# autosome-ru/pasio

Hardware: NVIDIA B200
Metric: whole-contig segmentation throughput, default pasio pipeline (nt/s); DP cell updates/s in dp_cells_per_s (higher is better)
Workload: dtype f64

## Files before the change

### include/pasio_b200.h

```cpp
#ifndef PASIO_B200_H
#define PASIO_B200_H

#include <stdint.h>

#ifdef __cplusplus
extern "C" {
#endif

typedef struct pasio_ctx pasio_ctx;

typedef enum pasio_status {
    PASIO_OK = 0,
    PASIO_E_CUDA = -1,
    PASIO_E_ARG = -2,
    PASIO_E_COUNTS = -3,
    PASIO_E_CANDIDATES = -4,
    PASIO_E_TABLE_TOO_SHORT = -5,
    PASIO_E_STATE = -6,
    PASIO_E_TOO_LARGE = -7,
    PASIO_E_NOMEM = -8
} pasio_status;

enum { PASIO_TAB_LOG = 0,
       PASIO_TAB_LGAMMA = 1,
// ... 26 lines not shown

int pasio_contig_load(pasio_ctx *ctx, const int64_t *counts, int64_t n,
                      const int64_t *offsets, int64_t n_contigs);
int pasio_contig_load_rle(pasio_ctx *ctx, const int64_t *starts, const int64_t *values,
                          int64_t n_runs, const int64_t *offsets, int64_t n_contigs);
int pasio_contig_load_round(pasio_ctx *ctx, const int64_t *counts, int64_t n, int64_t window_size,
                            int64_t window_shift, int constraint, int64_t *n_in, int64_t *n_out, int64_t *cells);

int pasio_contig_load_device(pasio_ctx *ctx, const int64_t *d_counts_device, int64_t n,
                             const int64_t *offsets, int64_t n_contigs);
int pasio_contig_info(const pasio_ctx *ctx, int64_t *n, int64_t *total_count, int64_t *n_contigs);
int pasio_cumsum_at(pasio_ctx *ctx, const int64_t *positions, int64_t m, int64_t *out);

int pasio_candidates_set(pasio_ctx *ctx, const int64_t *cands, int64_t m);
int pasio_candidates_count(const pasio_ctx *ctx, int64_t *m);
int pasio_candidates_download(pasio_ctx *ctx, int64_t *out, int64_t capacity, int64_t *m);

int pasio_filter_candidates(pasio_ctx *ctx, int constraint, int64_t *n_in, int64_t *n_out);

int pasio_round(pasio_ctx *ctx, int64_t window_size, int64_t window_shift, int constraint,
                int64_t *n_in, int64_t *n_out, int64_t *cells);
int pasio_round_stats(const pasio_ctx *ctx, int64_t *cells, int64_t *cells_skipped);
int pasio_round_certify_stats(const pasio_ctx *ctx, int64_t *passed, int64_t *fell_back, int64_t *resume_rows_sum);
int pasio_exact_task_plan(int64_t n_candidates, int lag, int nblock, int32_t *triples, int64_t cap, int64_t *n_tasks);
int pasio_upload_stats(const pasio_ctx *ctx, int64_t *wire_bytes);
int pasio_set_tuning(pasio_ctx *ctx, int key, int value);
int pasio_rounds(pasio_ctx *ctx, int64_t window_size, int64_t window_shift, int constraint,
                 int64_t max_rounds, int64_t *rounds_done, int64_t *n_out, int64_t *cells,
                 int64_t *sizes, int64_t sizes_cap);
int pasio_set_penalties(pasio_ctx *ctx, const double *split_number_penalty, int64_t n_split_number_penalty,
                        double first_column_refund, const double *length_penalty, int64_t n_length_penalty);

int pasio_square_split(pasio_ctx *ctx, int64_t *out_splits, int64_t cap, int64_t *n_splits,
                       double *score, double *prefix_scores, int64_t *previous_splits);
int pasio_square_split_regularized(pasio_ctx *ctx, const double *length_penalty, int64_t n_length_penalty,
                                   const double *split_number_penalty, int64_t n_split_number_penalty,
                                   double first_column_refund, int64_t *out_splits, int64_t cap, int64_t *n_splits,
                                   double *score, double *prefix_scores, int64_t *previous_splits);
int pasio_suffix_scores(pasio_ctx *ctx, int64_t stop, double *out);

int pasio_segment_scores(pasio_ctx *ctx, double *scores, int64_t *segment_counts,
                         double *mean_counts, double *logfac_cumsum, int64_t capacity,
                         int64_t *n_segments);

int pasio_segment_scores_sum(pasio_ctx *ctx, double *total);

// ... 32 lines not shown
```

### pasio_b200/_native.py

```python
import ctypes
import os
import threading

import numpy as np

_HERE = os.path.dirname(os.path.abspath(__file__))
LIB_PATH = os.environ.get('PASIO_B200_LIB') or os.path.join(_HERE, 'libpasio_b200.so')

OK = 0
E_CUDA, E_ARG, E_COUNTS, E_CANDIDATES, E_TABLE_TOO_SHORT, E_STATE, E_TOO_LARGE, E_NOMEM = range(-1, -9, -1)
TAB_LOG, TAB_LGAMMA, TAB_LGAMMA_ALPHA = 0, 1, 2
CONSTRAINTS = {'none': 0, 'zeros': 1, 'constants': 2}
TUNE = {'window_prune': 0, 'window_phases': 1, 'exact_prune': 2, 'exact_lag': 3, 'exact_ring': 4, 'logfac_exact': 5,
        'window_speculate': 6, 'upload_narrow': 7,
        'logfac_eager': 8, 'exact_nblock': 9, 'window_certify': 10}
TIMING_FAMILIES = ['scan', 'window_dp', 'compact', 'exact_dp', 'score', 'h2d', 'd2h']

_i64 = ctypes.c_int64
_i64p = ctypes.POINTER(ctypes.c_int64)
_f64p = ctypes.POINTER(ctypes.c_double)
_vp = ctypes.c_void_p

SIGNATURES = {
    'pasio_ctx_create': (ctypes.c_int, [ctypes.c_int, ctypes.POINTER(_vp)]),
    'pasio_ctx_destroy': (ctypes.c_int, [_vp]),
    'pasio_last_error': (ctypes.c_char_p, [_vp]),
    'pasio_abi_version': (ctypes.c_int, []),
    'pasio_set_params': (ctypes.c_int, [_vp, ctypes.c_int, ctypes.c_double, ctypes.c_double, ctypes.c_double]),
    'pasio_table_upload': (ctypes.c_int, [_vp, ctypes.c_int, _f64p, _i64]),
    'pasio_table_need': (ctypes.c_int, [_vp, _i64p, _i64p, _i64p]),
    'pasio_contig_load': (ctypes.c_int, [_vp, _i64p, _i64, _i64p, _i64]),
    'pasio_contig_load_round': (ctypes.c_int, [_vp, _i64p, _i64, _i64, _i64, ctypes.c_int, _i64p, _i64p, _i64p]),
    'pasio_contig_load_rle': (ctypes.c_int, [_vp, _i64p, _i64p, _i64, _i64p, _i64]),
    'pasio_contig_load_device': (ctypes.c_int, [_vp, _vp, _i64, _i64p, _i64]),
    'pasio_contig_info': (ctypes.c_int, [_vp, _i64p, _i64p, _i64p]),
    'pasio_cumsum_at': (ctypes.c_int, [_vp, _i64p, _i64, _i64p]),
    'pasio_candidates_set': (ctypes.c_int, [_vp, _i64p, _i64]),
    'pasio_candidates_count': (ctypes.c_int, [_vp, _i64p]),
    'pasio_candidates_download': (ctypes.c_int, [_vp, _i64p, _i64, _i64p]),
    'pasio_filter_candidates': (ctypes.c_int, [_vp, ctypes.c_int, _i64p, _i64p]),
    'pasio_round': (ctypes.c_int, [_vp, _i64, _i64, ctypes.c_int, _i64p, _i64p, _i64p]),
    'pasio_round_stats': (ctypes.c_int, [_vp, _i64p, _i64p]),
    'pasio_round_certify_stats': (ctypes.c_int, [_vp, _i64p, _i64p, _i64p]),
    'pasio_exact_task_plan': (ctypes.c_int, [_i64, ctypes.c_int, ctypes.c_int, ctypes.POINTER(ctypes.c_int32), _i64, _i64p]),
    'pasio_upload_stats': (ctypes.c_int, [_vp, _i64p]),
    'pasio_set_tuning': (ctypes.c_int, [_vp, ctypes.c_int, ctypes.c_int]),
    'pasio_rounds': (ctypes.c_int, [_vp, _i64, _i64, ctypes.c_int, _i64, _i64p, _i64p, _i64p, _i64p, _i64]),
    'pasio_set_penalties': (ctypes.c_int, [_vp, _f64p, _i64, ctypes.c_double, _f64p, _i64]),
    'pasio_square_split': (ctypes.c_int, [_vp, _i64p, _i64, _i64p, _f64p, _f64p, _i64p]),
    'pasio_square_split_regularized': (ctypes.c_int, [_vp, _f64p, _i64, _f64p, _i64, ctypes.c_double, _i64p, _i64, _i64p, _f64p,
                                                     _f64p, _i64p]),
    'pasio_suffix_scores': (ctypes.c_int, [_vp, _i64, _f64p]),
    'pasio_segment_scores': (ctypes.c_int, [_vp, _f64p, _i64p, _f64p, _f64p, _i64, _i64p]),
    'pasio_segment_scores_sum': (ctypes.c_int, [_vp, _f64p]),
    'pasio_segment_lmm': (ctypes.c_int, [_vp, _f64p, _i64, _f64p]),
    'pasio_logfac_prefetch': (ctypes.c_int, [_vp]),
    'pasio_host_alloc': (ctypes.c_int, [_i64, ctypes.POINTER(_vp)]),
    'pasio_host_free': (ctypes.c_int, [_vp]),
    'pasio_bedgraph_count_lines': (_i64, [ctypes.c_void_p, _i64]),
    'pasio_bedgraph_parse': (ctypes.c_int, [ctypes.c_void_p, _i64, _i64, _i64p, _i64p, _i64p, _i64p,
                                            ctypes.POINTER(ctypes.c_int32), ctypes.POINTER(ctypes.c_uint8), _i64p, _i64p]),
    'pasio_bedgraph_runs': (_i64, [_i64p, _i64p, _i64p, ctypes.POINTER(ctypes.c_uint8), _i64, ctypes.c_int, _i64p, _i64p, _i64p,
                                   _i64p, _i64p]),
    'pasio_format_segments': (_i64, [ctypes.c_char_p, _i64, _i64p, _i64, _f64p, _f64p, ctypes.c_int,
                                     ctypes.c_char_p, _i64]),
    'pasio_format_segments_batch': (_i64, [ctypes.c_char_p, _i64p, _i64p, _i64p, _i64, _i64p, _f64p, _f64p, ctypes.c_int,
# ... 312 lines not shown
        self._sync_penalties()
        self._retry(lambda: self.lib.pasio_round(self.ctx, window_size, window_shift, CONSTRAINTS[constraint],
                                                 ctypes.byref(n_in), ctypes.byref(n_out), ctypes.byref(cells)))
        return n_in.value, n_out.value, cells.value

    def set_tuning(self, key, value):
        self._check(self.lib.pasio_set_tuning(self.ctx, TUNE[key], int(value)))

    def upload_stats(self):
        b = _i64(0)
        self._check(self.lib.pasio_upload_stats(self.ctx, ctypes.byref(b)))
        return b.value

    def round_stats(self):
        a, b = _i64(0), _i64(0)
        self._check(self.lib.pasio_round_stats(self.ctx, ctypes.byref(a), ctypes.byref(b)))
        return a.value, b.value

    def round_certify_stats(self):
        a, b, c = _i64(0), _i64(0), _i64(0)
        self._check(self.lib.pasio_round_certify_stats(self.ctx, ctypes.byref(a), ctypes.byref(b), ctypes.byref(c)))
        return a.value, b.value, c.value

    def rounds(self, window_size, window_shift, constraint, num_rounds=None, first=None):
        n, _, _ = self.info()
        limit = max(1, n if num_rounds is None else num_rounds)
        self._cands_obj = None
        sizes, cells_total = [], 0
        if first is not None:
            sizes.append(first[0])
            cells_total += first[2]
            limit -= 1
            if first[0] == first[1] or limit == 0:
                return sizes, self.candidate_count(), cells_total
        while limit > 0:
            done, n_out, cells = _i64(0), _i64(0), _i64(0)
            buf = np.zeros(64, dtype=np.int64)
            step = min(limit, 64)
            self._sync_penalties()
            rc = self.lib.pasio_rounds(self.ctx, window_size, window_shift, CONSTRAINTS[constraint], step,
                                       ctypes.byref(done), ctypes.byref(n_out), ctypes.byref(cells),
                                       _ptr(buf, ctypes.c_int64), len(buf))
            sizes.extend(buf[:done.value].tolist())
            cells_total += cells.value
            limit -= done.value
            if rc == E_TABLE_TOO_SHORT:
# ... 224 lines not shown
```

### pasio_b200/csrc/api.cu

```cuda
#include "common.cuh"

#include <algorithm>
#include <thread>
#include <atomic>
#include <chrono>
#include <memory>
#include <cstdarg>
#include <cstdlib>
#include <cstdio>
#include <cstring>

static thread_local std::string g_create_error;

int pasio_fail(pasio_ctx *ctx, int code, const char *fmt, ...)
{
    char buf[512];
    va_list ap;
    va_start(ap, fmt);
    vsnprintf(buf, sizeof buf, fmt, ap);
    va_end(ap);
    if (ctx) ctx->err = buf; else g_create_error = buf;
    return code;
}

// ... 364 lines not shown
        return pasio_fail(nullptr, PASIO_E_ARG, "device %d out of range (have %d)", device, count);
    cudaDeviceProp prop;
    e = cudaGetDeviceProperties(&prop, device);
    if (e != cudaSuccess) return pasio_fail(nullptr, PASIO_E_CUDA, "cudaGetDeviceProperties: %s", cudaGetErrorString(e));
    if (prop.major != 10)
        return pasio_fail(nullptr, PASIO_E_CUDA, "device %d is sm_%d%d; this library is built for sm_100a only",
                          device, prop.major, prop.minor);
    e = cudaSetDevice(device);
    if (e != cudaSuccess) return pasio_fail(nullptr, PASIO_E_CUDA, "cudaSetDevice: %s", cudaGetErrorString(e));
    pasio_ctx *ctx = new pasio_ctx();
    ctx->device = device;
    ctx->sm_count = prop.multiProcessorCount;
    ctx->smem_optin = (int)prop.sharedMemPerBlockOptin;
    int prio_lo = 0, prio_hi = 0;
    cudaDeviceGetStreamPriorityRange(&prio_lo, &prio_hi);
    if (cudaStreamCreateWithPriority(&ctx->stream, cudaStreamNonBlocking, prio_hi) != cudaSuccess ||
        cudaStreamCreateWithPriority(&ctx->stream2, cudaStreamNonBlocking, 0) != cudaSuccess ||
        cudaStreamCreateWithFlags(&ctx->stream_copy, cudaStreamNonBlocking) != cudaSuccess ||
        cudaStreamCreateWithPriority(&ctx->stream_lx, cudaStreamNonBlocking, 0) != cudaSuccess ||
        cudaEventCreateWithFlags(&ctx->ev_lx0, cudaEventDisableTiming) != cudaSuccess ||
        cudaEventCreateWithFlags(&ctx->ev_lx1, cudaEventDisableTiming) != cudaSuccess ||
        cudaEventCreateWithFlags(&ctx->ev_fork, cudaEventDisableTiming) != cudaSuccess ||
        cudaEventCreateWithFlags(&ctx->ev_join, cudaEventDisableTiming) != cudaSuccess ||
        cudaMallocHost((void **)&ctx->h_scalars, 20 * sizeof(i64)) != cudaSuccess ||
        pasio_reserve(ctx, ctx->scalars, 20 * sizeof(i64)) != PASIO_OK) {
        g_create_error = "context allocation failed: " + ctx->err;
        delete ctx;
        return PASIO_E_CUDA;
    }
    memset(ctx->h_scalars, 0, 20 * sizeof(i64));
    auto env_int = [](const char *name, int dflt) { const char *v = getenv(name); return v ? atoi(v) : dflt; };
    ctx->tune[PASIO_TUNE_WINDOW_PRUNE] = env_int("PASIO_WD_PRUNE", 1);
    ctx->tune[PASIO_TUNE_WINDOW_PHASES] = env_int("PASIO_WD_PHASES", 1);
    ctx->tune[PASIO_TUNE_EXACT_PRUNE] = env_int("PASIO_XD_PRUNE", 1);
    ctx->tune[PASIO_TUNE_EXACT_LAG] = env_int("PASIO_XD_LAG", 5);
    ctx->tune[PASIO_TUNE_EXACT_RING] = env_int("PASIO_XD_RING", 1);
    ctx->tune[PASIO_TUNE_LOGFAC_EXACT] = env_int("PASIO_B200_EXACT_LMM", 1);
    ctx->tune[PASIO_TUNE_WINDOW_SPECULATE] = env_int("PASIO_WD_SPECULATE", 1);
    ctx->tune[PASIO_TUNE_UPLOAD_NARROW] = env_int("PASIO_B200_UPLOAD_NARROW", 1);
    ctx->tune[PASIO_TUNE_LOGFAC_EAGER] = env_int("PASIO_B200_LOGFAC_EAGER", 0);
    ctx->tune[PASIO_TUNE_EXACT_NBLOCK] = env_int("PASIO_XD_NBLOCK", 3);
    ctx->tune[PASIO_TUNE_WINDOW_CERTIFY] = env_int("PASIO_WD_CERTIFY", 1);
    if (ctx->tune[PASIO_TUNE_EXACT_LAG] < 3 || ctx->tune[PASIO_TUNE_EXACT_LAG] > 5) ctx->tune[PASIO_TUNE_EXACT_LAG] = 5;
    *out = ctx;
    return PASIO_OK;
}

extern "C" int pasio_ctx_destroy(pasio_ctx *ctx)
{
    if (!ctx) return PASIO_OK;
    cudaSetDevice(ctx->device);
    cudaStreamSynchronize(ctx->stream);
    drop_borrowed_counts(ctx);
// ... 384 lines not shown
    if (ctx->h_scalars[1]) return pasio_fail(ctx, PASIO_E_COUNTS, "counts must be >= 0");
    ctx->total = ctx->h_scalars[0];
    ctx->max_count = ctx->h_scalars[2];
    ctx->have_contig = true;
    if (eager) {
        CUDA_TRY(ctx, cudaEventRecord(ctx->ev_lx1, ctx->stream_lx));
        ctx->logfac_ready = true;
        ctx->logfac_is_exact = true;
        ctx->logfac_pending = true;
        ctx->logfac_eager = true;
    }
    PASIO_TRY(launch_boundary_ranks(ctx));
    ctx->h_brank = ctx->h_bounds;
    if (n_in) *n_in = ctx->m;
    if (n_out) *n_out = ctx->m;
    if (cells) *cells = 0;
    if (table_rc != PASIO_OK) return table_rc;

    const int nxt = 1 - ctx->cur;
    PASIO_TRY(pasio_reserve(ctx, ctx->cand[nxt], (size_t)ctx->m * 4));
    i64 m_new = 0;
    PASIO_TRY(launch_compact_keepbits(ctx, nxt, &m_new));
    PASIO_TRY(d2h(ctx, ctx->h_scalars + 10, ctx->scalars.as<i64>() + 10, 24));
    PASIO_TRY(d2h(ctx, ctx->h_scalars + 16, ctx->scalars.as<i64>() + 16, 24));
    if (cells) *cells = ctx->h_scalars[10];
    ctx->last_cells = ctx->h_scalars[10];
    ctx->last_cells_skipped = ctx->h_scalars[12];
    for (int k = 0; k < 3; ++k) ctx->last_certify[k] = ctx->h_scalars[16 + k];
    ctx->prev_round_in = ctx->m;
    ctx->prev_round_out = m_new;
    ctx->cur = nxt;
    ctx->implicit_all = false;
    ctx->m = m_new;
    if (n_out) *n_out = m_new;
    return refresh_boundary_ranks(ctx);
}

extern "C" int pasio_contig_info(const pasio_ctx *ctx, int64_t *n, int64_t *total_count, int64_t *n_contigs)
{
    if (!ctx || !ctx->have_contig) return PASIO_E_STATE;
    if (n) *n = ctx->n;
    if (total_count) *total_count = ctx->total;
    if (n_contigs) *n_contigs = ctx->n_contigs;
    return PASIO_OK;
}

extern "C" int pasio_cumsum_at(pasio_ctx *ctx, const int64_t *positions, int64_t m, int64_t *out)
{
    NEED_CTX(ctx);
    if (!ctx->have_contig) return pasio_fail(ctx, PASIO_E_STATE, "no contig loaded");
    if (m < 0 || !out) return pasio_fail(ctx, PASIO_E_ARG, "bad arguments");
// ... 163 lines not shown
    static const bool debug = getenv("PASIO_DEBUG") != nullptr;
    if (debug)
        fprintf(stderr, "[pasio_round] n=%lld contigs=%lld m=%lld implicit=%d nwin=%lld size=%lld shift=%lld max_span=%lld max_cnt=%lld ntab=%lld,%lld,%lld\n",
                (long long)ctx->n, (long long)ctx->n_contigs, (long long)ctx->m, (int)ctx->implicit_all, (long long)nwin,
                (long long)window_size, (long long)window_shift, (long long)max_span, (long long)max_cnt,
                (long long)ctx->ntab[0], (long long)ctx->ntab[1], (long long)ctx->ntab[2]);
    if (max_cnt > ctx->total || max_span > ctx->n)
        return pasio_fail(ctx, PASIO_E_CUDA, "internal inconsistency before the window DP: window count %lld / span %lld exceed "
                          "contig total %lld / length %lld (m=%lld, implicit=%d, windows=%lld)", (long long)max_cnt,
                          (long long)max_span, (long long)ctx->total, (long long)ctx->n, (long long)ctx->m,
                          (int)ctx->implicit_all, (long long)nwin);
    PASIO_TRY(check_dp_tables(ctx, max_span, max_cnt, true));

    const size_t bit_bytes = (size_t)((ctx->n + 1 + 31) / 32 + 2) * 4;
    CUDA_TRY(ctx, cudaMemsetAsync(ctx->keepbits.p, 0, bit_bytes, ctx->stream));
    if (penalties_on(ctx)) PASIO_TRY(launch_window_dp_reg(ctx, nwin, (int)window_size, (int)window_shift, constraint));
    else PASIO_TRY(launch_window_dp(ctx, nwin, (int)window_size, (int)window_shift, constraint));

    const int nxt = 1 - ctx->cur;
    PASIO_TRY(pasio_reserve(ctx, ctx->cand[nxt], (size_t)ctx->m * 4));
    i64 m_new = 0;
    PASIO_TRY(launch_compact_keepbits(ctx, nxt, &m_new));
    PASIO_TRY(d2h(ctx, ctx->h_scalars + 10, ctx->scalars.as<i64>() + 10, 24));
    PASIO_TRY(d2h(ctx, ctx->h_scalars + 16, ctx->scalars.as<i64>() + 16, 24));
    if (cells) *cells = ctx->h_scalars[10];
    ctx->last_cells = ctx->h_scalars[10];
    ctx->last_cells_skipped = ctx->h_scalars[12];
    for (int k = 0; k < 3; ++k) ctx->last_certify[k] = ctx->h_scalars[16 + k];
    ctx->prev_round_in = ctx->m;
    ctx->prev_round_out = m_new;
    ctx->cur = nxt;
    ctx->implicit_all = false;
    ctx->m = m_new;
    if (n_out) *n_out = m_new;
    return refresh_boundary_ranks(ctx);
}

extern "C" int pasio_rounds(pasio_ctx *ctx, int64_t window_size, int64_t window_shift, int constraint,
                            int64_t max_rounds, int64_t *rounds_done, int64_t *n_out, int64_t *cells,
                            int64_t *sizes, int64_t sizes_cap)
{
    NEED_CTX(ctx);
    if (!ctx->have_contig) return pasio_fail(ctx, PASIO_E_STATE, "no contig loaded");
    i64 limit = max_rounds <= 0 ? ctx->n : max_rounds;
    if (limit < 1) limit = 1;
    i64 done = 0, total_cells = 0;
    int rc = PASIO_OK;
    while (done < limit) {
        int64_t a = 0, b = 0, c = 0;
        rc = pasio_round(ctx, window_size, window_shift, constraint, &a, &b, &c);
        if (rc != PASIO_OK) break;
// ... 9 lines not shown
}

extern "C" int pasio_upload_stats(const pasio_ctx *ctx, int64_t *wire_bytes)
{
    if (!ctx || !wire_bytes) return PASIO_E_ARG;
    *wire_bytes = ctx->last_wire_bytes;
    return PASIO_OK;
}

extern "C" int pasio_round_stats(const pasio_ctx *ctx, int64_t *cells, int64_t *cells_skipped)
{
    if (!ctx) return PASIO_E_ARG;
    if (cells) *cells = ctx->last_cells;
    if (cells_skipped) *cells_skipped = ctx->last_cells_skipped;
    return PASIO_OK;
}

extern "C" int pasio_round_certify_stats(const pasio_ctx *ctx, int64_t *passed, int64_t *fell_back, int64_t *resume_rows_sum)
{
    if (!ctx) return PASIO_E_ARG;
    if (passed) *passed = ctx->last_certify[0];
    if (fell_back) *fell_back = ctx->last_certify[1];
    if (resume_rows_sum) *resume_rows_sum = ctx->last_certify[2];
    return PASIO_OK;
}

extern "C" int pasio_set_tuning(pasio_ctx *ctx, int key, int value)
{
    if (!ctx) return PASIO_E_ARG;
    if (key < 0 || key >= PASIO_TUNE_COUNT) return pasio_fail(ctx, PASIO_E_ARG, "unknown tuning key %d", key);
    if (key == PASIO_TUNE_EXACT_LAG && (value < 3 || value > 5)) return pasio_fail(ctx, PASIO_E_ARG, "exact lag must be 3, 4 or 5");
    ctx->tune[key] = value;
    if (key == PASIO_TUNE_LOGFAC_EXACT) {
        if (ctx->logfac_pending) { cudaStreamSynchronize(ctx->stream_lx); ctx->logfac_pending = false; }
        ctx->logfac_ready = false;
        ctx->logfac_eager = false;
    }
    return PASIO_OK;
}

static int finish_square_split(pasio_ctx *ctx, i64 N, int64_t *out_splits, int64_t cap, int64_t *n_splits, double *score,
                               double *prefix_scores, int64_t *previous_splits)
{
    if (score) PASIO_TRY(d2h(ctx, score, ctx->dpP.as<double>() + (N - 1), 8));
    if (prefix_scores) PASIO_TRY(d2h(ctx, prefix_scores, ctx->dpP.p, (size_t)N * 8));
    if (previous_splits) {
// ... 335 lines not shown
```

### pasio_b200/csrc/common.cuh

```cuda
#pragma once

#include <cuda_runtime.h>
#include <stdint.h>
#include <string>
#include <vector>

#include "../../include/pasio_b200.h"

typedef long long i64;
typedef unsigned long long u64;

#define PASIO_ABI_VERSION 1

struct DevBuf {
    void *p = nullptr;
    size_t bytes = 0;
    template <typename T> T *as() const { return reinterpret_cast<T *>(p); }
};

enum TimingFamily { TF_SCAN = 0, TF_WINDOW_DP = 1, TF_COMPACT = 2, TF_EXACT_DP = 3, TF_SCORE = 4,
                    TF_H2D = 5, TF_D2H = 6, TF_COUNT = 7 };

struct TimedSpan { int family; cudaEvent_t a, b; };

// ... 54 lines not shown

    DevBuf win_st, win_en;
    DevBuf win_flags;
    DevBuf win_small, win_medium, win_large;
    i64 n_small = 0, n_medium = 0, n_large = 0;
    i64 n_large_p1 = 0;
    std::vector<int32_t> h_win_st, h_win_en, h_brank;

    DevBuf blocksum, tilestate, scalars, dpL, dpC, dpP, dpPrev, dpPart, dpPartArg, dpMark, dpJump, fscan, logfac_full;
    DevBuf xpRing, xpRec, xpTasks, regLR, regNR;

    bool pen_num = false, pen_len = false;
    DevBuf penNR, penLR;
    i64 n_pen_nr = 0, n_pen_lr = 0;
    double pen_refund = 0.0;
    DevBuf lxPos, lxSum, lxFirst, lxState;
    i64 lx_terms = 0;
    i64 scan_tiles_done = 0;

    int tune[PASIO_TUNE_COUNT];
    i64 *h_scalars = nullptr;

    i64 last_cells = 0, last_cells_skipped = 0;
    i64 last_certify[3] = {0, 0, 0};
    i64 prev_round_in = 0, prev_round_out = 0;
    std::vector<i64> pw_leaf_start;
    i64 pw_n = -1;
    std::vector<double> pw_leaf_sum;

    bool timing = false;
    std::vector<TimedSpan> spans;
    std::vector<cudaEvent_t> event_pool;
    double fam_ms[TF_COUNT] = {0};
    i64 fam_launches[TF_COUNT] = {0};
};

int pasio_fail(pasio_ctx *ctx, int code, const char *fmt, ...);
int pasio_reserve(pasio_ctx *ctx, DevBuf &b, size_t bytes);

#define CUDA_TRY(ctx, call)                                                                     \
    do {                                                                                        \
        cudaError_t e__ = (call);                                                               \
        if (e__ != cudaSuccess)                                                                 \
            return pasio_fail((ctx), PASIO_E_CUDA, "%s failed: %s (%s:%d)", #call,              \
                              cudaGetErrorString(e__), __FILE__, __LINE__);                     \
    } while (0)

// ... 92 lines not shown
```

### pasio_b200/csrc/window_dp.cu

```cuda
#include "dp_core.cuh"
#include "bound.cuh"
#include <cstdio>
#include <cstdlib>

namespace {

constexpr int WD_THREADS = 256;
constexpr int WD_WARPS = WD_THREADS / 32;
constexpr int WD_FARW = WD_WARPS - 1;
constexpr int NEAR_Q = 4;
constexpr int PR_CB = 32;
constexpr int PR_FB = 8;
constexpr int PR_MIN_N = 256;
constexpr int PR_DENSE = 28;

#ifdef PASIO_WD_PROF
__device__ unsigned long long g_wd_prof[16];
struct ProfAcc { long long t0; long long a0, a1, a2, a3, a4, a5, a6, a7; };
#define PROF_DECL ProfAcc prof = {clock64(), 0, 0, 0, 0, 0, 0, 0, 0}
__device__ __forceinline__ long long prof_clock()
{
    unsigned dummy;
    long long t;
    asm volatile("ld.volatile.shared.u32 %0, [%1];" : "=r"(dummy) : "r"(0u) : "memory");
    asm volatile("mov.u64 %0, %%clock64;" : "=l"(t) : "r"(dummy) : "memory");
    return t;
}
#define PROF_T(i) do { const long long t1__ = prof_clock(); prof.a##i += t1__ - prof.t0; prof.t0 = t1__; } while (0)
#define PROF_FLUSH do { if (threadIdx.x == 0 || threadIdx.x == 32) { unsigned long long *g__ = g_wd_prof + (threadIdx.x ? 8 : 0); \
    atomicAdd(g__ + 0, (unsigned long long)prof.a0); atomicAdd(g__ + 1, (unsigned long long)prof.a1); \
    atomicAdd(g__ + 2, (unsigned long long)prof.a2); atomicAdd(g__ + 3, (unsigned long long)prof.a3); \
    atomicAdd(g__ + 4, (unsigned long long)prof.a4); atomicAdd(g__ + 5, (unsigned long long)prof.a5); \
    atomicAdd(g__ + 6, (unsigned long long)prof.a6); atomicAdd(g__ + 7, (unsigned long long)prof.a7); } \
    prof.a0 = prof.a1 = prof.a2 = prof.a3 = prof.a4 = prof.a5 = prof.a6 = prof.a7 = 0; } while (0)
#define PROF_ARGS , ProfAcc &prof
#define PROF_PASS , prof
#else
// ... 311 lines not shown
                const int row = (t & 3) * 8 + k * 4 + rr;
                sPartV[(t >> 2) * 32 + row] = best;
                sPartA[(t >> 2) * 32 + row] = arg;
            }
        }
    }
#pragma unroll
    for (int kk = 0; kk < NK; ++kk) {
        const int k = w7 + kk * NW;
        if (k < lane && jb + lane < N) sTri[k * DP_JB + lane] = w[kk];
    }
}

__device__ __forceinline__ void build_coarse_record(int jb, const ColRec *sCol, CoarseRec *rec, double tilt_scale_c,
                                                    double tilt_scale_l)
{
    const ColRec me = sCol[jb + (threadIdx.x & 31)];
    fit_column_record(me.C, me.L, me.P, rec, tilt_scale_c, tilt_scale_l);
}

constexpr int CT_RB = 16;

template <bool AI>
__device__ __forceinline__ int certify_window(const WinDpParams &p, int N, ColRec *sCol, CoarseRec *sCoarse, const double *sScal0,
                                              double *sScal1, double *sT, float4 *sRowG, double *sLbAbs, int *sSkip,
                                              unsigned short *sL1, int *sFail, int *sL1Count, double tilt_c, double tilt_l,
                                              u64 &skipped)
{
    const int tid = threadIdx.x, lane = tid & 31, warp = tid >> 5;
    const int nrb = (N - 1 + DP_JB - 1) / DP_JB;
    if (tid == 0) { *sFail = N; *sL1Count = 0; }
    if (tid < CT_RB) sSkip[tid] = 0;
    for (int kg = 0; kg < nrb; kg += CT_RB) {
        const int r0 = 1 + DP_JB * kg, r1 = min(N, r0 + DP_JB * CT_RB), kge = min(nrb, kg + CT_RB);
        for (int j = r0 + tid; j < r1; j += WD_THREADS) {
            const int2 me = col_lc(sCol, j), bf = col_lc(sCol, j - 1);
            sT[j - r0] = self_score<AI>(bf.y, bf.x, make_row<AI>(me.y, me.x, p.alpha_int, p.alpha), p.gtab, p.ltab);
        }
        __syncthreads();
        if (tid == 0) {
            double P = sCol[r0 - 1].P, mx = *sScal1;
            for (int j = r0; j < r1; ++j) {
                const double t = __dadd_rn(sT[j - r0], P);
                P = __dadd_rn(t, p.pen);
                sT[j - r0] = t;
                sCol[j].P = P;
                mx = fmax(mx, fabs(P));
            }
            *sScal1 = mx;
        }
        __syncthreads();
        for (int k = kg + warp; k < kge; k += WD_WARPS) {
            const int jb = 1 + DP_JB * k;
            if (jb + DP_JB <= N) build_coarse_record(jb, sCol, sCoarse + k, tilt_c, tilt_l);
            const bool valid = jb + lane < N;
            const int j = min(jb + lane, N - 1);
            const double T = sT[j - r0];
            const int2 me = col_lc(sCol, j);
            const RowConst<AI> rme = make_row<AI>(me.y, me.x, p.alpha_int, p.alpha);
            const int c0 = k == 0 ? 0 : jb - DP_JB;
            const int dmax = j - c0, dmax_w = __reduce_max_sync(0xffffffffu, dmax);
            bool ok = fabs(T) < 1e30;
            constexpr int UN = 4;
            for (int d = 2; d <= dmax_w; d += UN) {
                double t[UN];
#pragma unroll
                for (int u = 0; u < UN; ++u) {
                    const ColRec c = sCol[max(j - d - u, 0)];
                    t[u] = d + u <= dmax ? __dadd_rn(self_score<AI>(c.C, c.L, rme, p.gtab, p.ltab), c.P) : -INFINITY;
                }
// ... 274 lines not shown
        if (PRUNE && tid == 0) {
            const ColRec z = sCol[N - 1];
            const int x = z.C + (AI ? p.alpha_int : 0);
            sScal[0] = fabs(__ldg(p.gtab + x)) + ((double)z.C + p.alpha) * fabs(__ldg(p.ltab + z.L)) + 1.0;
            sScal[1] = 0.0;
            sScal[2] = (double)z.C + p.alpha;
            sScal[3] = (double)z.L;
        }
        auto finish_block = [&](int jb) {
            if (jb + DP_JB <= N) build_coarse_record(jb, sCol, sCoarse + (jb - 1) / PR_CB, sScal[2], sScal[3]);
            double ab = jb + lane < N ? fabs(sCol[jb + lane].P) : 0.0;
#pragma unroll
            for (int off = 16; off > 0; off >>= 1) ab = fmax(ab, __shfl_xor_sync(0xffffffffu, ab, off));
            if (lane == 0) sScal[1] = fmax(sScal[1], ab);
        };
        auto far_delta = [&]() { return (sScal[0] + sScal[1] + fabs(p.pen) * DP_JB) * 5.684341886080802e-14; };
        auto prepare_rows = [&](int jbn) {
            const int par = ((jbn - 1) / DP_JB) & 1;
            const double delta_path = (sScal[0] + sScal[1] + fabs(p.pen) * DP_JB) * 1.8189894035458565e-12;
            compute_row_lb<AI>(jbn - DP_JB, jbn, N, sCol, sRow + 32 * par, sScal + 4 + par, delta_path, p.pen, p.gtab, p.ltab,
                               p.alpha_int, p.alpha);
            if (lane == 0) { sListCount[4 * par] = 0; sListCount[4 * par + 1] = 0; sListCount[4 * par + 2] = 0; }
        };
        auto run_far = [&](int jbf) {
            const int kf = (jbf - 1) / DP_JB, par = kf & 1;
            skipped += far_pass<AI>(jbf, N, kf - 1, sCol, sCoarse, sRow + 32 * par, sScal[4 + par], sList, sList + capr,
                                    sList + capr + capr / PR_CB + 8, sListCount + 4 * par, sFarV + (par * WD_FARW + warp - 1) * 32,
                                    sFarA + (par * WD_FARW + warp - 1) * 32,
                                    far_delta(), p.gtab, p.ltab, p.alpha_int, p.alpha PROF_PASS);
        };
        int jb = 1;
        const bool pipelined = PRUNE && N > PR_MIN_N && p.cand != nullptr;
        bool passed = false;
        if (pipelined && p.certify) {
            __syncthreads();
            const int f = certify_window<AI>(p, N, sCol, sCoarse, sScal, sScal + 1, sFarV, reinterpret_cast<float4 *>(sTri), sPartV,
                                             sPartA, sList, sMisc + 2, sMisc + 3, sScal[2], sScal[3], skipped);
            passed = f >= N;
            const int kf = (f - 1) / DP_JB, res = passed || kf < 2 ? 1 : 1 + DP_JB * kf;
            for (int j = 1 + tid; j < res; j += WD_THREADS) sPrev[j] = (unsigned short)(j - 1);
            if (warp == 0 && !passed) {
                double ab = 0.0;
                for (int j = 1 + lane; j < res; j += 32) ab = fmax(ab, fabs(sCol[j].P));
#pragma unroll
                for (int off = 16; off > 0; off >>= 1) ab = fmax(ab, __shfl_xor_sync(0xffffffffu, ab, off));
                if (lane == 0) sScal[1] = ab;
            }
            if (tid == 0) {
                atomicAdd(p.certify_stats + (passed ? 0 : 1), 1ull);
                if (res > 1) atomicAdd(p.certify_stats + 2, (u64)(res - 1));
            }
            jb = passed ? N : res;
            __syncthreads();
        }
        for (; jb < N && (!pipelined || jb < 1 + 2 * DP_JB); jb += DP_JB) {
            dp_block_step<AI, WD_WARPS, U, RPL>(jb, N, 0, sCol, sPrev, nullptr, sPartV, sPartA, sTri,
                                                p.gtab, p.ltab, p.alpha_int, p.alpha, p.pen, -INFINITY, 0, 0);
            if (pipelined && warp == 0) finish_block(jb);
        }
        PROF_T(6);
        if (pipelined && jb < N) {
            int spec_wait = 0, spec_back = 1;
            if (warp == 0) prepare_rows(jb);
            __syncthreads();
            if (warp > 0) run_far(jb);
            else if (jb + DP_JB < N) prepare_rows(jb + DP_JB);
            __syncthreads();
            for (; jb < N; jb += DP_JB) {
                const int k = (jb - 1) / DP_JB, buf = k & 1;
                near_tri_farwarps<AI, WD_WARPS>(warp, jb, N, sCol, sPartV, sPartA, sTri, p.gtab, p.ltab, p.alpha_int, p.alpha);
                PROF_T(1);
                __syncthreads();
                PROF_T(6);
                if (warp == 0) {
                    double fbest = -INFINITY;
                    int farg = 0;
#pragma unroll
                    for (int w2 = 0; w2 < WD_FARW; ++w2) {
                        const double v = sFarV[(buf * WD_FARW + w2) * 32 + lane];
                        const int a = sFarA[(buf * WD_FARW + w2) * 32 + lane];
                        if (v > fbest || (v == fbest && a < farg)) { fbest = v; farg = a; }
                    }
                    const double ib = jb + lane < N ? fbest : -INFINITY;
                    const int ia = jb + lane < N ? farg : 0;
                    bool resolved = false;
                    if (p.speculate && spec_wait == 0) {
                        resolved = block_chain_speculative<NEAR_Q>(jb, N, sCol, sPrev, sPartV, sPartA, sTri, p.pen, ib, ia);
                        if (resolved) spec_back = 1;
                        else { spec_wait = spec_back; spec_back = min(spec_back * 2, 16); }
                    } else if (spec_wait > 0) {
                        --spec_wait;
                    }
                    if (!resolved) block_chain<NEAR_Q>(jb, N, sCol, sPrev, nullptr, sPartV, sPartA, sTri, p.pen, ib, ia, 0, nullptr);
                    __syncwarp();
                    finish_block(jb);
                    if (jb + 2 * DP_JB < N) prepare_rows(jb + 2 * DP_JB);
                } else if (jb + DP_JB < N) {
                    run_far(jb + DP_JB);
                }
                PROF_T(2);
                __syncthreads();
                PROF_T(7);
            }
        }

        for (int k = tid; k < N; k += WD_THREADS) sMark[k] = passed || k == N - 1;
        __syncthreads();
        unsigned short *ja = sPrev, *jb2 = sJump;
        for (int reach = passed ? N : 1; reach < N; reach <<= 1) {
            for (int k = tid; k < N; k += WD_THREADS)
                if (sMark[k]) sMark[ja[k]] = 1;
            for (int k = tid; k < N; k += WD_THREADS) jb2[k] = ja[ja[k]];
            __syncthreads();
            unsigned short *t = ja; ja = jb2; jb2 = t;
        }
        int every = N == nq;
        for (int k = tid; k < N; k += WD_THREADS) {
            if (sMark[k]) {
                const i64 pos = first + sCol[k].L;
                atomicOr(p.keepbits + (pos >> 5), 1u << (pos & 31));
            } else {
                every = 0;
            }
        }
        if (!second && p.skip_covered && p.n_p1 < p.nwin) {
            __threadfence();
            every = __syncthreads_and(every);
// ... 190 lines not shown
    p.cgc = cur_cand_cg(ctx);
    p.cpbits = ctx->cpbits.as<uint32_t>();
    p.keepbits = ctx->keepbits.as<uint32_t>();
    p.gtab = ctx->tab[ctx->alpha_is_int ? PASIO_TAB_LGAMMA : PASIO_TAB_LGAMMA_ALPHA].as<double>();
    p.ltab = ctx->tab[PASIO_TAB_LOG].as<double>();
    p.constraint = constraint;
    p.alpha_int = (int)ctx->alpha_int;
    p.alpha = ctx->alpha;
    p.pen = ctx->pen;
    i64 cap = (i64)wsize + 1;
    if (cap > ctx->m) cap = ctx->m;
    if (cap > 8192 || window_smem_bytes((int)cap) > (size_t)ctx->smem_optin)
        return pasio_fail(ctx, PASIO_E_TOO_LARGE, "window of %lld candidates does not fit one CTA's shared memory (max %d)",
                          (long long)cap, window_dp_max_candidates(ctx));
    p.cap = (int)cap;
    p.cells = ctx->scalars.as<u64>() + 10;
    p.cells_skipped = ctx->scalars.as<u64>() + 12;
    p.work_counter = ctx->scalars.as<unsigned>() + 2 * 11;
    p.w_begin = w_begin;
    p.certify_stats = ctx->scalars.as<u64>() + 16;
    if (keep_cell_counters) CUDA_TRY(ctx, cudaMemsetAsync(ctx->scalars.as<u64>() + 11, 0, 8, ctx->stream));
    else {
        CUDA_TRY(ctx, cudaMemsetAsync(ctx->scalars.as<u64>() + 10, 0, 24, ctx->stream));
        CUDA_TRY(ctx, cudaMemsetAsync(p.certify_stats, 0, 24, ctx->stream));
    }
    CUDA_TRY(ctx, cudaMemsetAsync(ctx->scalars.as<u64>() + 15, 0, 8, ctx->stream));

    static const int small_env = getenv("PASIO_WD_SMALL") ? atoi(getenv("PASIO_WD_SMALL")) : 1;
    const int phase_env = ctx->tune[PASIO_TUNE_WINDOW_PHASES];
    const bool use_lists = small_env && ctx->n_small + ctx->n_medium + ctx->n_large == nwin;
    const i64 n_small = use_lists ? ctx->n_small : 0, n_medium = use_lists ? ctx->n_medium : 0;
    const i64 n_large = use_lists ? ctx->n_large : nwin;
    p.list = use_lists ? ctx->win_large.as<int32_t>() : nullptr;
    p.nwin = n_large;
    p.list_len = nwin;
    p.n_p1 = use_lists ? ctx->n_large_p1 : n_large;
    p.skip_covered = phase_env;
    p.speculate = ctx->tune[PASIO_TUNE_WINDOW_SPECULATE];
    const int certify_env = ctx->tune[PASIO_TUNE_WINDOW_CERTIFY];
    p.certify = certify_env >= 2 ||
                (certify_env == 1 && ctx->prev_round_in > 0 && (ctx->prev_round_in - ctx->prev_round_out) * 100 < ctx->prev_round_in);
    p.done_flags = ctx->win_flags.as<unsigned char>();
    p.p1_stride = wshift > 0 && wsize / wshift > 1 ? wsize / wshift : 1;
    if (!use_lists) p.skip_covered = 0;
    ctx->n_small = ctx->n_medium = ctx->n_large = ctx->n_large_p1 = -1;
    TimingScope ts_all(ctx, TF_WINDOW_DP, 0);
    const bool fork = n_small + n_medium > 0 && n_small + n_medium <= 64;
    const bool serial_small = n_small + n_medium > 64;
    if (fork) CUDA_TRY(ctx, cudaEventRecord(ctx->ev_fork, ctx->stream));

    auto launch_small = [&](auto kern, const int32_t *list, i64 n, int nwarps, int ctas, size_t smem_bytes, unsigned *counter,
                            cudaStream_t stream) -> int {
        if (n <= 0) return PASIO_OK;
        WinDpParams ps = p;
        ps.list = list;
        ps.nwin = n;
        ps.n_p1 = n;
        ps.work_counter = counter;
        CUDA_TRY(ctx, cudaFuncSetAttribute(kern, cudaFuncAttributeMaxDynamicSharedMemorySize, (int)smem_bytes));
        int resident = ctas;
        CUDA_TRY(ctx, cudaOccupancyMaxActiveBlocksPerMultiprocessor(&resident, kern, nwarps * 32, smem_bytes));
        if (resident < 1) resident = 1;
        if (resident > ctas) resident = ctas;
        i64 g = (n + nwarps - 1) / nwarps;
// ... 76 lines not shown
```

Baseline: 6.352 billion.

## Re-enter window certification after DP blocks return to identity predecessors

After a failed certification, the pipelined window DP now watches for a block whose predecessors are all the immediately preceding column. When it sees one, it leaves the pipeline and re-runs the certification from that block, up to eight times per window, so the remaining exact DP can be skipped. The certify serial prefix loop is also unrolled by eight, and the default certify trigger is loosened so it fires when the previous round removed under 20% of candidates instead of under 1%. New counters record recheck starts, rechecks reaching the end, and blocks computed after a failure. The costs are extra warp votes, an extra barrier check per block, pipeline restarts, and running certification on more rounds where it may fail.

```diff
diff --git a/include/pasio_b200.h b/include/pasio_b200.h
--- a/include/pasio_b200.h
+++ b/include/pasio_b200.h
@@ -72,6 +72,7 @@
                 int64_t *n_in, int64_t *n_out, int64_t *cells);
 int pasio_round_stats(const pasio_ctx *ctx, int64_t *cells, int64_t *cells_skipped);
 int pasio_round_certify_stats(const pasio_ctx *ctx, int64_t *passed, int64_t *fell_back, int64_t *resume_rows_sum);
+int pasio_round_recheck_stats(const pasio_ctx *ctx, int64_t *started, int64_t *reached_end, int64_t *blocks_after_fail);
 int pasio_exact_task_plan(int64_t n_candidates, int lag, int nblock, int32_t *triples, int64_t cap, int64_t *n_tasks);
 int pasio_upload_stats(const pasio_ctx *ctx, int64_t *wire_bytes);
 int pasio_set_tuning(pasio_ctx *ctx, int key, int value);
diff --git a/pasio_b200/_native.py b/pasio_b200/_native.py
--- a/pasio_b200/_native.py
+++ b/pasio_b200/_native.py
@@ -42,6 +42,7 @@
     'pasio_round': (ctypes.c_int, [_vp, _i64, _i64, ctypes.c_int, _i64p, _i64p, _i64p]),
     'pasio_round_stats': (ctypes.c_int, [_vp, _i64p, _i64p]),
     'pasio_round_certify_stats': (ctypes.c_int, [_vp, _i64p, _i64p, _i64p]),
+    'pasio_round_recheck_stats': (ctypes.c_int, [_vp, _i64p, _i64p, _i64p]),
     'pasio_exact_task_plan': (ctypes.c_int, [_i64, ctypes.c_int, ctypes.c_int, ctypes.POINTER(ctypes.c_int32), _i64, _i64p]),
     'pasio_upload_stats': (ctypes.c_int, [_vp, _i64p]),
     'pasio_set_tuning': (ctypes.c_int, [_vp, ctypes.c_int, ctypes.c_int]),
@@ -400,6 +401,11 @@
         self._check(self.lib.pasio_round_certify_stats(self.ctx, ctypes.byref(a), ctypes.byref(b), ctypes.byref(c)))
         return a.value, b.value, c.value
 
+    def round_recheck_stats(self):
+        a, b, c = _i64(0), _i64(0), _i64(0)
+        self._check(self.lib.pasio_round_recheck_stats(self.ctx, ctypes.byref(a), ctypes.byref(b), ctypes.byref(c)))
+        return a.value, b.value, c.value
+
     def rounds(self, window_size, window_shift, constraint, num_rounds=None, first=None):
         n, _, _ = self.info()
         limit = max(1, n if num_rounds is None else num_rounds)
diff --git a/pasio_b200/csrc/api.cu b/pasio_b200/csrc/api.cu
--- a/pasio_b200/csrc/api.cu
+++ b/pasio_b200/csrc/api.cu
@@ -410,13 +410,13 @@
         cudaEventCreateWithFlags(&ctx->ev_lx1, cudaEventDisableTiming) != cudaSuccess ||
         cudaEventCreateWithFlags(&ctx->ev_fork, cudaEventDisableTiming) != cudaSuccess ||
         cudaEventCreateWithFlags(&ctx->ev_join, cudaEventDisableTiming) != cudaSuccess ||
-        cudaMallocHost((void **)&ctx->h_scalars, 20 * sizeof(i64)) != cudaSuccess ||
-        pasio_reserve(ctx, ctx->scalars, 20 * sizeof(i64)) != PASIO_OK) {
+        cudaMallocHost((void **)&ctx->h_scalars, 24 * sizeof(i64)) != cudaSuccess ||
+        pasio_reserve(ctx, ctx->scalars, 24 * sizeof(i64)) != PASIO_OK) {
         g_create_error = "context allocation failed: " + ctx->err;
         delete ctx;
         return PASIO_E_CUDA;
     }
-    memset(ctx->h_scalars, 0, 20 * sizeof(i64));
+    memset(ctx->h_scalars, 0, 24 * sizeof(i64));
     auto env_int = [](const char *name, int dflt) { const char *v = getenv(name); return v ? atoi(v) : dflt; };
     ctx->tune[PASIO_TUNE_WINDOW_PRUNE] = env_int("PASIO_WD_PRUNE", 1);
     ctx->tune[PASIO_TUNE_WINDOW_PHASES] = env_int("PASIO_WD_PHASES", 1);
@@ -847,11 +847,11 @@
     i64 m_new = 0;
     PASIO_TRY(launch_compact_keepbits(ctx, nxt, &m_new));
     PASIO_TRY(d2h(ctx, ctx->h_scalars + 10, ctx->scalars.as<i64>() + 10, 24));
-    PASIO_TRY(d2h(ctx, ctx->h_scalars + 16, ctx->scalars.as<i64>() + 16, 24));
+    PASIO_TRY(d2h(ctx, ctx->h_scalars + 16, ctx->scalars.as<i64>() + 16, 48));
     if (cells) *cells = ctx->h_scalars[10];
     ctx->last_cells = ctx->h_scalars[10];
     ctx->last_cells_skipped = ctx->h_scalars[12];
-    for (int k = 0; k < 3; ++k) ctx->last_certify[k] = ctx->h_scalars[16 + k];
+    for (int k = 0; k < 6; ++k) ctx->last_certify[k] = ctx->h_scalars[16 + k];
     ctx->prev_round_in = ctx->m;
     ctx->prev_round_out = m_new;
     ctx->cur = nxt;
@@ -1061,11 +1061,11 @@
     i64 m_new = 0;
     PASIO_TRY(launch_compact_keepbits(ctx, nxt, &m_new));
     PASIO_TRY(d2h(ctx, ctx->h_scalars + 10, ctx->scalars.as<i64>() + 10, 24));
-    PASIO_TRY(d2h(ctx, ctx->h_scalars + 16, ctx->scalars.as<i64>() + 16, 24));
+    PASIO_TRY(d2h(ctx, ctx->h_scalars + 16, ctx->scalars.as<i64>() + 16, 48));
     if (cells) *cells = ctx->h_scalars[10];
     ctx->last_cells = ctx->h_scalars[10];
     ctx->last_cells_skipped = ctx->h_scalars[12];
-    for (int k = 0; k < 3; ++k) ctx->last_certify[k] = ctx->h_scalars[16 + k];
+    for (int k = 0; k < 6; ++k) ctx->last_certify[k] = ctx->h_scalars[16 + k];
     ctx->prev_round_in = ctx->m;
     ctx->prev_round_out = m_new;
     ctx->cur = nxt;
@@ -1121,6 +1121,15 @@
     if (passed) *passed = ctx->last_certify[0];
     if (fell_back) *fell_back = ctx->last_certify[1];
     if (resume_rows_sum) *resume_rows_sum = ctx->last_certify[2];
+    return PASIO_OK;
+}
+
+extern "C" int pasio_round_recheck_stats(const pasio_ctx *ctx, int64_t *started, int64_t *reached_end, int64_t *blocks_after_fail)
+{
+    if (!ctx) return PASIO_E_ARG;
+    if (started) *started = ctx->last_certify[3];
+    if (reached_end) *reached_end = ctx->last_certify[4];
+    if (blocks_after_fail) *blocks_after_fail = ctx->last_certify[5];
     return PASIO_OK;
 }
 
diff --git a/pasio_b200/csrc/common.cuh b/pasio_b200/csrc/common.cuh
--- a/pasio_b200/csrc/common.cuh
+++ b/pasio_b200/csrc/common.cuh
@@ -100,7 +100,7 @@
     i64 *h_scalars = nullptr;
 
     i64 last_cells = 0, last_cells_skipped = 0;
-    i64 last_certify[3] = {0, 0, 0};
+    i64 last_certify[6] = {0, 0, 0, 0, 0, 0};
     i64 prev_round_in = 0, prev_round_out = 0;
     std::vector<i64> pw_leaf_start;
     i64 pw_n = -1;
diff --git a/pasio_b200/csrc/window_dp.cu b/pasio_b200/csrc/window_dp.cu
--- a/pasio_b200/csrc/window_dp.cu
+++ b/pasio_b200/csrc/window_dp.cu
@@ -13,6 +13,7 @@
 constexpr int PR_FB = 8;
 constexpr int PR_MIN_N = 256;
 constexpr int PR_DENSE = 28;
+constexpr int WD_RECHECKS = 8;
 
 #ifdef PASIO_WD_PROF
 __device__ unsigned long long g_wd_prof[16];
@@ -370,16 +371,16 @@
 constexpr int CT_RB = 16;
 
 template <bool AI>
-__device__ __forceinline__ int certify_window(const WinDpParams &p, int N, ColRec *sCol, CoarseRec *sCoarse, const double *sScal0,
-                                              double *sScal1, double *sT, float4 *sRowG, double *sLbAbs, int *sSkip,
-                                              unsigned short *sL1, int *sFail, int *sL1Count, double tilt_c, double tilt_l,
-                                              u64 &skipped)
+__device__ __forceinline__ int certify_window(const WinDpParams &p, int N, int kb0, ColRec *sCol, CoarseRec *sCoarse,
+                                              const double *sScal0, double *sScal1, double *sT, float4 *sRowG, double *sLbAbs,
+                                              int *sSkip, unsigned short *sL1, int *sFail, int *sL1Count, double tilt_c,
+                                              double tilt_l, u64 &skipped)
 {
     const int tid = threadIdx.x, lane = tid & 31, warp = tid >> 5;
     const int nrb = (N - 1 + DP_JB - 1) / DP_JB;
     if (tid == 0) { *sFail = N; *sL1Count = 0; }
     if (tid < CT_RB) sSkip[tid] = 0;
-    for (int kg = 0; kg < nrb; kg += CT_RB) {
+    for (int kg = kb0; kg < nrb; kg += CT_RB) {
         const int r0 = 1 + DP_JB * kg, r1 = min(N, r0 + DP_JB * CT_RB), kge = min(nrb, kg + CT_RB);
         for (int j = r0 + tid; j < r1; j += WD_THREADS) {
             const int2 me = col_lc(sCol, j), bf = col_lc(sCol, j - 1);
@@ -387,13 +388,22 @@
         }
         __syncthreads();
         if (tid == 0) {
+            constexpr int CB_U = 8;
             double P = sCol[r0 - 1].P, mx = *sScal1;
-            for (int j = r0; j < r1; ++j) {
-                const double t = __dadd_rn(sT[j - r0], P);
-                P = __dadd_rn(t, p.pen);
-                sT[j - r0] = t;
-                sCol[j].P = P;
-                mx = fmax(mx, fabs(P));
+            for (int j0 = r0; j0 < r1; j0 += CB_U) {
+                double s[CB_U];
+#pragma unroll
+                for (int u = 0; u < CB_U; ++u) s[u] = j0 + u < r1 ? sT[j0 + u - r0] : 0.0;
+#pragma unroll
+                for (int u = 0; u < CB_U; ++u) {
+                    if (j0 + u < r1) {
+                        const double t = __dadd_rn(s[u], P);
+                        P = __dadd_rn(t, p.pen);
+                        sT[j0 + u - r0] = t;
+                        sCol[j0 + u].P = P;
+                        mx = fmax(mx, fabs(P));
+                    }
+                }
             }
             *sScal1 = mx;
         }
@@ -714,9 +724,9 @@
                                p.alpha_int, p.alpha);
             if (lane == 0) { sListCount[4 * par] = 0; sListCount[4 * par + 1] = 0; sListCount[4 * par + 2] = 0; }
         };
-        auto run_far = [&](int jbf) {
+        auto run_far = [&](int jbf) -> unsigned {
             const int kf = (jbf - 1) / DP_JB, par = kf & 1;
-            skipped += far_pass<AI>(jbf, N, kf - 1, sCol, sCoarse, sRow + 32 * par, sScal[4 + par], sList, sList + capr,
+            return (unsigned)far_pass<AI>(jbf, N, kf - 1, sCol, sCoarse, sRow + 32 * par, sScal[4 + par], sList, sList + capr,
                                     sList + capr + capr / PR_CB + 8, sListCount + 4 * par, sFarV + (par * WD_FARW + warp - 1) * 32,
                                     sFarA + (par * WD_FARW + warp - 1) * 32,
                                     far_delta(), p.gtab, p.ltab, p.alpha_int, p.alpha PROF_PASS);
@@ -724,77 +734,104 @@
         int jb = 1;
         const bool pipelined = PRUNE && N > PR_MIN_N && p.cand != nullptr;
         bool passed = false;
-        if (pipelined && p.certify) {
-            __syncthreads();
-            const int f = certify_window<AI>(p, N, sCol, sCoarse, sScal, sScal + 1, sFarV, reinterpret_cast<float4 *>(sTri), sPartV,
-                                             sPartA, sList, sMisc + 2, sMisc + 3, sScal[2], sScal[3], skipped);
-            passed = f >= N;
-            const int kf = (f - 1) / DP_JB, res = passed || kf < 2 ? 1 : 1 + DP_JB * kf;
-            for (int j = 1 + tid; j < res; j += WD_THREADS) sPrev[j] = (unsigned short)(j - 1);
-            if (warp == 0 && !passed) {
-                double ab = 0.0;
-                for (int j = 1 + lane; j < res; j += 32) ab = fmax(ab, fabs(sCol[j].P));
-#pragma unroll
-                for (int off = 16; off > 0; off >>= 1) ab = fmax(ab, __shfl_xor_sync(0xffffffffu, ab, off));
-                if (lane == 0) sScal[1] = ab;
-            }
-            if (tid == 0) {
-                atomicAdd(p.certify_stats + (passed ? 0 : 1), 1ull);
-                if (res > 1) atomicAdd(p.certify_stats + 2, (u64)(res - 1));
-            }
-            jb = passed ? N : res;
-            __syncthreads();
-        }
-        for (; jb < N && (!pipelined || jb < 1 + 2 * DP_JB); jb += DP_JB) {
-            dp_block_step<AI, WD_WARPS, U, RPL>(jb, N, 0, sCol, sPrev, nullptr, sPartV, sPartA, sTri,
-                                                p.gtab, p.ltab, p.alpha_int, p.alpha, p.pen, -INFINITY, 0, 0);
-            if (pipelined && warp == 0) finish_block(jb);
-        }
-        PROF_T(6);
-        if (pipelined && jb < N) {
-            int spec_wait = 0, spec_back = 1;
-            if (warp == 0) prepare_rows(jb);
-            __syncthreads();
-            if (warp > 0) run_far(jb);
-            else if (jb + DP_JB < N) prepare_rows(jb + DP_JB);
-            __syncthreads();
-            for (; jb < N; jb += DP_JB) {
-                const int k = (jb - 1) / DP_JB, buf = k & 1;
-                near_tri_farwarps<AI, WD_WARPS>(warp, jb, N, sCol, sPartV, sPartA, sTri, p.gtab, p.ltab, p.alpha_int, p.alpha);
-                PROF_T(1);
+        int kcheck = pipelined && p.certify ? 0 : -1, rechecks = 0, pipe_blocks = 0;
+        do {
+            if (kcheck >= 0) {
                 __syncthreads();
-                PROF_T(6);
-                if (warp == 0) {
-                    double fbest = -INFINITY;
-                    int farg = 0;
-#pragma unroll
-                    for (int w2 = 0; w2 < WD_FARW; ++w2) {
-                        const double v = sFarV[(buf * WD_FARW + w2) * 32 + lane];
-                        const int a = sFarA[(buf * WD_FARW + w2) * 32 + lane];
-                        if (v > fbest || (v == fbest && a < farg)) { fbest = v; farg = a; }
+                const int f = certify_window<AI>(p, N, kcheck, sCol, sCoarse, sScal, sScal + 1, sFarV, reinterpret_cast<float4 *>(sTri),
+                                                 sPartV, sPartA, sList, sMisc + 2, sMisc + 3, sScal[2], sScal[3], skipped);
+                const bool first_check = kcheck == 0;
+                if (first_check) passed = f >= N;
+                const int kf = (f - 1) / DP_JB, res = passed ? 1 : f >= N ? N : kf < 2 ? 1 : 1 + DP_JB * kf;
+                for (int j = 1 + DP_JB * kcheck + tid; j < res; j += WD_THREADS) sPrev[j] = (unsigned short)(j - 1);
+                if (warp == 0 && f < N) {
+                    double ab = 0.0;
+                    for (int j = 1 + lane; j < res; j += 32) ab = fmax(ab, fabs(sCol[j].P));
+#pragma unroll
+                    for (int off = 16; off > 0; off >>= 1) ab = fmax(ab, __shfl_xor_sync(0xffffffffu, ab, off));
+                    if (lane == 0) sScal[1] = ab;
+                }
+                if (tid == 0) {
+                    if (first_check) {
+                        atomicAdd(p.certify_stats + (passed ? 0 : 1), 1ull);
+                        if (res > 1) atomicAdd(p.certify_stats + 2, (u64)(res - 1));
+                    } else {
+                        atomicAdd(p.certify_stats + 3, 1ull);
+                        if (f >= N) atomicAdd(p.certify_stats + 4, 1ull);
                     }
-                    const double ib = jb + lane < N ? fbest : -INFINITY;
-                    const int ia = jb + lane < N ? farg : 0;
-                    bool resolved = false;
-                    if (p.speculate && spec_wait == 0) {
-                        resolved = block_chain_speculative<NEAR_Q>(jb, N, sCol, sPrev, sPartV, sPartA, sTri, p.pen, ib, ia);
-                        if (resolved) spec_back = 1;
-                        else { spec_wait = spec_back; spec_back = min(spec_back * 2, 16); }
-                    } else if (spec_wait > 0) {
-                        --spec_wait;
+                }
+                jb = f >= N ? N : res;
+                kcheck = -1;
+                __syncthreads();
+            }
+            for (; jb < N && (!pipelined || jb < 1 + 2 * DP_JB); jb += DP_JB) {
+                dp_block_step<AI, WD_WARPS, U, RPL>(jb, N, 0, sCol, sPrev, nullptr, sPartV, sPartA, sTri,
+                                                    p.gtab, p.ltab, p.alpha_int, p.alpha, p.pen, -INFINITY, 0, 0);
+                if (pipelined && warp == 0) finish_block(jb);
+                ++pipe_blocks;
+            }
+            PROF_T(6);
+            if (pipelined && jb < N) {
+                int spec_wait = 0, spec_back = 1;
+                unsigned far_sk = 0;
+                const bool may_exit = p.certify && rechecks < WD_RECHECKS;
+                if (warp == 0) prepare_rows(jb);
+                __syncthreads();
+                if (warp > 0) far_sk = run_far(jb);
+                else if (jb + DP_JB < N) prepare_rows(jb + DP_JB);
+                __syncthreads();
+                for (; jb < N; jb += DP_JB) {
+                    const int k = (jb - 1) / DP_JB, buf = k & 1;
+                    skipped += far_sk;
+                    far_sk = 0;
+                    ++pipe_blocks;
+                    near_tri_farwarps<AI, WD_WARPS>(warp, jb, N, sCol, sPartV, sPartA, sTri, p.gtab, p.ltab, p.alpha_int, p.alpha);
+                    PROF_T(1);
+                    __syncthreads();
+                    PROF_T(6);
+                    if (warp == 0) {
+                        double fbest = -INFINITY;
+                        int farg = 0;
+#pragma unroll
+                        for (int w2 = 0; w2 < WD_FARW; ++w2) {
+                            const double v = sFarV[(buf * WD_FARW + w2) * 32 + lane];
+                            const int a = sFarA[(buf * WD_FARW + w2) * 32 + lane];
+                            if (v > fbest || (v == fbest && a < farg)) { fbest = v; farg = a; }
+                        }
+                        const double ib = jb + lane < N ? fbest : -INFINITY;
+                        const int ia = jb + lane < N ? farg : 0;
+                        bool resolved = false;
+                        if (p.speculate && spec_wait == 0) {
+                            resolved = block_chain_speculative<NEAR_Q>(jb, N, sCol, sPrev, sPartV, sPartA, sTri, p.pen, ib, ia);
+                            if (resolved) spec_back = 1;
+                            else { spec_wait = spec_back; spec_back = min(spec_back * 2, 16); }
+                        } else if (spec_wait > 0) {
+                            --spec_wait;
+                        }
+                        if (!resolved) block_chain<NEAR_Q>(jb, N, sCol, sPrev, nullptr, sPartV, sPartA, sTri, p.pen, ib, ia, 0, nullptr);
+                        __syncwarp();
+                        finish_block(jb);
+                        if (jb + 2 * DP_JB < N) prepare_rows(jb + 2 * DP_JB);
+                        if (may_exit) {
+                            const bool keep = jb + DP_JB < N && __all_sync(0xffffffffu, sPrev[jb + lane] == jb + lane - 1);
+                            if (lane == 0) sMisc[12] = keep;
+                        }
+                    } else if (jb + DP_JB < N) {
+                        far_sk = run_far(jb + DP_JB);
                     }
-                    if (!resolved) block_chain<NEAR_Q>(jb, N, sCol, sPrev, nullptr, sPartV, sPartA, sTri, p.pen, ib, ia, 0, nullptr);
-                    __syncwarp();
-                    finish_block(jb);
-                    if (jb + 2 * DP_JB < N) prepare_rows(jb + 2 * DP_JB);
-                } else if (jb + DP_JB < N) {
-                    run_far(jb + DP_JB);
-                }
-                PROF_T(2);
-                __syncthreads();
-                PROF_T(7);
-            }
-        }
+                    PROF_T(2);
+                    __syncthreads();
+                    PROF_T(7);
+                    if (may_exit && sMisc[12]) {
+                        kcheck = k + 1;
+                        ++rechecks;
+                        jb += DP_JB;
+                        break;
+                    }
+                }
+            }
+        } while (kcheck >= 0);
+        if (tid == 0 && p.certify && pipelined && !passed) atomicAdd(p.certify_stats + 5, (u64)pipe_blocks);
 
         for (int k = tid; k < N; k += WD_THREADS) sMark[k] = passed || k == N - 1;
         __syncthreads();
@@ -1031,7 +1068,7 @@
     if (keep_cell_counters) CUDA_TRY(ctx, cudaMemsetAsync(ctx->scalars.as<u64>() + 11, 0, 8, ctx->stream));
     else {
         CUDA_TRY(ctx, cudaMemsetAsync(ctx->scalars.as<u64>() + 10, 0, 24, ctx->stream));
-        CUDA_TRY(ctx, cudaMemsetAsync(p.certify_stats, 0, 24, ctx->stream));
+        CUDA_TRY(ctx, cudaMemsetAsync(p.certify_stats, 0, 48, ctx->stream));
     }
     CUDA_TRY(ctx, cudaMemsetAsync(ctx->scalars.as<u64>() + 15, 0, 8, ctx->stream));
 
@@ -1048,7 +1085,7 @@
     p.speculate = ctx->tune[PASIO_TUNE_WINDOW_SPECULATE];
     const int certify_env = ctx->tune[PASIO_TUNE_WINDOW_CERTIFY];
     p.certify = certify_env >= 2 ||
-                (certify_env == 1 && ctx->prev_round_in > 0 && (ctx->prev_round_in - ctx->prev_round_out) * 100 < ctx->prev_round_in);
+                (certify_env == 1 && ctx->prev_round_in > 0 && (ctx->prev_round_in - ctx->prev_round_out) * 5 < ctx->prev_round_in);
     p.done_flags = ctx->win_flags.as<unsigned char>();
     p.p1_stride = wshift > 0 && wsize / wshift > 1 ? wsize / wshift : 1;
     if (!use_lists) p.skip_covered = 0;
```

After: 6.612 billion (median of 6 runs). +4.1%, better.
